# mdolab/adflow

Measured on AMD Instinct MI355X. Metric: Mcells*residual-evals/s, higher is better.
Workload: dtype f64

## Files before the change

### adflow_amd/capi.py

```python
from __future__ import annotations

import ctypes
import os
from ctypes import POINTER, c_char_p, c_double, c_int, c_int8, c_int32, c_uint, c_void_p
from typing import Optional

import numpy as np

from . import params as P

_HERE = os.path.dirname(os.path.abspath(__file__))
LIB_PATH = os.path.join(_HERE, "lib", "libadflow_gpu.so")
MAX_RK = 8


class AdflowOpts(ctypes.Structure):
    _fields_ = [
        ("equations", c_int32), ("turbModel", c_int32), ("turbProd", c_int32),
        ("useQCR", c_int32), ("useRotationSA", c_int32), ("useft2SA", c_int32),
        ("spaceDiscr", c_int32), ("spaceDiscrCoarse", c_int32), ("limiter", c_int32), ("orderTurb", c_int32),
        ("dirScaling", c_int32),
        ("smoother", c_int32), ("nRKStages", c_int32), ("resAveraging", c_int32), ("nSubiterations", c_int32),
        ("nSubIterTurb", c_int32),
        ("groundLevel", c_int32),
# ... 76 lines not shown
        ("rotMatrix", c_double * 9), ("rotCenter", c_double * 3), ("translation", c_double * 3),
        ("nHalos", c_int32), ("reserved", c_int32), ("block", c_void_p), ("indices", c_void_p),
    ]


class AdflowCommPattern(ctypes.Structure):
    _fields_ = [
        ("ncopy", c_int32),
        ("donorBlock", c_void_p), ("donorIndices", c_void_p), ("haloBlock", c_void_p), ("haloIndices", c_void_p),
        ("nProcSend", c_int32), ("sendProc", c_void_p), ("nsendCum", c_void_p), ("sendBlock", c_void_p),
        ("sendIndices", c_void_p),
        ("nProcRecv", c_int32), ("recvProc", c_void_p), ("nrecvCum", c_void_p), ("recvBlock", c_void_p),
        ("recvIndices", c_void_p),
    ]


BC_CALLBACK = ctypes.CFUNCTYPE(None, c_int, c_int)

(ARR_W, ARR_P, ARR_GAMMA, ARR_RLV, ARR_REV, ARR_DW, ARR_FW, ARR_DTL, ARR_RADI, ARR_RADJ, ARR_RADK, ARR_AA,
 ARR_NODAL_GRADS, ARR_WN, ARR_PN, ARR_W1, ARR_P1, ARR_WR, ARR_VOL, ARR_SI, ARR_SJ, ARR_SK, ARR_X, ARR_D2WALL) = range(1, 25)

JAC_PC, JAC_FROZEN_TURB, JAC_TURB_ONLY, JAC_VISC_PC, JAC_USE_AD = 1, 2, 4, 8, 16
RES_UPDATE_INTERMED, RES_FLOW, RES_TURB, RES_CLOSURES, RES_HALO = 1, 2, 4, 8, 16
RES_DISS_APPROX, RES_VISC_APPROX, RES_UPWIND_FIRST_ORDER, ANK_COUPLED = 32, 64, 128, 256
ANK_TURB, RES_APPROX_SA, RES_TURB_FIRST_ORDER, JAC_APPROX_SA = 512, 1024, 2048, 32

EXPORTS = [
    "adflow_gpu_init", "adflow_gpu_finalize", "adflow_gpu_last_error", "adflow_gpu_device_name",
    "adflow_gpu_comm_unique_id", "adflow_gpu_comm_init",
    "adflow_gpu_block_register", "adflow_gpu_block_release", "adflow_gpu_release_all", "adflow_gpu_upload_geometry", "adflow_gpu_upload_state",
    "adflow_gpu_download_state", "adflow_gpu_download_residual", "adflow_gpu_download_array",
    "adflow_gpu_upload_array", "adflow_gpu_set_options",
    "adflow_gpu_time_step", "adflow_gpu_initres", "adflow_gpu_residual", "adflow_gpu_block_res",
    "adflow_gpu_rk_smooth", "adflow_gpu_dadi_smooth", "adflow_gpu_halo_exchange", "adflow_gpu_res_norms",
    "adflow_gpu_sa_solve", "adflow_gpu_set_turb_bc_callback",
    "adflow_gpu_set_w_vec", "adflow_gpu_get_r_vec", "adflow_gpu_get_res", "adflow_gpu_nk_residual",
    "adflow_gpu_nk_residual_dev",
    "adflow_gpu_transfer_to_coarse", "adflow_gpu_transfer_to_fine", "adflow_gpu_mg_cycle",
    "adflow_gpu_comm_register", "adflow_gpu_comm_info", "adflow_gpu_halo_slot_info", "adflow_gpu_halo_pack", "adflow_gpu_halo_unpack",
    "adflow_gpu_halo_local_copy", "adflow_gpu_set_bc_callback", "adflow_gpu_bc_register", "adflow_gpu_apply_all_bc", "adflow_gpu_download_wall_stress", "adflow_gpu_abi_sizes2", "adflow_gpu_xhalo", "adflow_gpu_actuator_register", "adflow_gpu_comm_register_periodic", "adflow_gpu_coarse_coordinates", "adflow_gpu_exchange_coor",
    "adflow_gpu_upload_coordinates", "adflow_gpu_update_geometry", "adflow_gpu_reference_shock_sensor",
    "adflow_gpu_wall_distance_register", "adflow_gpu_update_wall_distances",
    "adflow_gpu_fd_jacobian", "adflow_gpu_release_workspace", "adflow_gpu_selftest_math", "adflow_gpu_jacobian_info", "adflow_gpu_download_jacobian", "adflow_gpu_download_jacobian_rows",
    "adflow_gpu_jacobian_mult", "adflow_gpu_jacobian_mult_dev",
    "adflow_gpu_pc_setup", "adflow_gpu_pc_info", "adflow_gpu_pc_apply", "adflow_gpu_pc_apply_dev", "adflow_gpu_pc_release", "adflow_gpu_pc_select",
    "adflow_gpu_pc_set_fill", "adflow_gpu_pc_info2",
    "adflow_gpu_gmres_solve", "adflow_gpu_gmres_solve_dev",
    "adflow_gpu_ank_set_w", "adflow_gpu_ank_set_w_dev", "adflow_gpu_ank_get_r", "adflow_gpu_ank_get_r_dev", "adflow_gpu_ank_time_step",
    "adflow_gpu_ank_download_time_step", "adflow_gpu_ank_pc_setup", "adflow_gpu_ank_set_base", "adflow_gpu_ank_set_base_dev",
    "adflow_gpu_ank_mult", "adflow_gpu_ank_mult_dev", "adflow_gpu_ank_last_h", "adflow_gpu_ank_solve", "adflow_gpu_ank_solve_dev",
    "adflow_gpu_ank_physicality_check", "adflow_gpu_ank_physicality_check_dev", "adflow_gpu_ank_release",
    "adflow_gpu_ank_download_time_step_turb", "adflow_gpu_ank_unsteady_res", "adflow_gpu_ank_unsteady_res_dev", "adflow_gpu_ank_select_base",
    "adflow_gpu_event_record", "adflow_gpu_event_elapsed_ms", "adflow_gpu_sync", "adflow_gpu_set_async",
    "adflow_gpu_abi_sizes", "adflow_gpu_set_tuning", "adflow_gpu_march_stats",
]

_libs = {}


class AdflowGpuError(RuntimeError):
    pass


def load(path: Optional[str] = None) -> ctypes.CDLL:
    path = path or LIB_PATH
    if path in _libs:
        return _libs[path]
    if not os.path.exists(path):
        raise AdflowGpuError(f"{path} not built: run `python -m adflow_amd.build` (no CPU fallback exists)")
    lib = ctypes.CDLL(path)
    lib.adflow_gpu_last_error.restype = c_char_p
    lib.adflow_gpu_init.argtypes = [c_int]
    lib.adflow_gpu_device_name.argtypes = [c_char_p, c_int]
    lib.adflow_gpu_block_register.argtypes = [c_int, c_int, c_int, POINTER(AdflowBlockDesc)]
    for n in ("adflow_gpu_block_release", "adflow_gpu_upload_geometry", "adflow_gpu_upload_state", "adflow_gpu_download_state",
              "adflow_gpu_download_residual"):
        getattr(lib, n).argtypes = [c_int, c_int, c_int]
    lib.adflow_gpu_download_array.argtypes = [c_int, c_int, c_int, c_int, c_void_p]
    lib.adflow_gpu_upload_array.argtypes = [c_int, c_int, c_int, c_int, c_void_p]
    lib.adflow_gpu_set_options.argtypes = [POINTER(AdflowOpts)]
    lib.adflow_gpu_time_step.argtypes = [c_int, c_int]
    lib.adflow_gpu_initres.argtypes = [c_int, c_int, c_int]
    lib.adflow_gpu_residual.argtypes = [c_int, c_int]
    lib.adflow_gpu_block_res.argtypes = [c_int, c_uint]
    lib.adflow_gpu_set_async.argtypes = [c_int]
    lib.adflow_gpu_bc_register.argtypes = [c_int, c_int, c_int, c_int, c_int, POINTER(AdflowBcSubface)]
    lib.adflow_gpu_apply_all_bc.argtypes = [c_int, c_int]
    lib.adflow_gpu_download_wall_stress.argtypes = [c_int, c_int, c_int, c_int, c_void_p, c_void_p]
    lib.adflow_gpu_upload_coordinates.argtypes = [c_int, c_int, c_int]
    lib.adflow_gpu_update_geometry.argtypes = [c_int]
    lib.adflow_gpu_xhalo.argtypes = [c_int]
    lib.adflow_gpu_actuator_register.argtypes = [c_int, POINTER(AdflowActuatorRegion)]
    lib.adflow_gpu_comm_register_periodic.argtypes = [c_int, c_int, c_int, POINTER(AdflowPeriodicData)]
    lib.adflow_gpu_coarse_coordinates.argtypes = [c_int]
    lib.adflow_gpu_exchange_coor.argtypes = [c_int]
    lib.adflow_gpu_reference_shock_sensor.argtypes = [c_int]
    lib.adflow_gpu_wall_distance_register.argtypes = [c_int, c_int, c_int, c_void_p, c_void_p]
    lib.adflow_gpu_update_wall_distances.argtypes = [c_int, c_void_p, ctypes.c_int64]
    lib.adflow_gpu_fd_jacobian.argtypes = [c_int, c_uint, c_double]
    lib.adflow_gpu_release_workspace.argtypes = [ctypes.POINTER(ctypes.c_int64)]
    lib.adflow_gpu_selftest_math.argtypes = [c_int, c_void_p, c_void_p, ctypes.c_int64, c_void_p, c_void_p]
    lib.adflow_gpu_jacobian_info.argtypes = [POINTER(ctypes.c_int32), POINTER(ctypes.c_int32), POINTER(ctypes.c_int32)]
    lib.adflow_gpu_download_jacobian.argtypes = [c_int, c_int, c_int, c_void_p]
    lib.adflow_gpu_download_jacobian_rows.argtypes = [c_int, c_int, c_int, c_void_p]
    lib.adflow_gpu_jacobian_mult.argtypes = [c_int, c_int, c_void_p, c_void_p, ctypes.c_long]
    lib.adflow_gpu_jacobian_mult_dev.argtypes = [c_int, c_int, c_void_p, c_void_p, ctypes.c_long]
    lib.adflow_gpu_pc_setup.argtypes = [c_int]
# ... 4 lines not shown
    for f in (lib.adflow_gpu_gmres_solve, lib.adflow_gpu_gmres_solve_dev):
        f.argtypes = [c_int, c_int, c_void_p, c_void_p, ctypes.c_long, c_int, c_int, c_double, c_double, c_int,
                      POINTER(c_int), POINTER(c_double), POINTER(c_double)]
    for f in (lib.adflow_gpu_ank_set_w, lib.adflow_gpu_ank_set_w_dev, lib.adflow_gpu_ank_get_r, lib.adflow_gpu_ank_get_r_dev,
              lib.adflow_gpu_ank_set_base, lib.adflow_gpu_ank_set_base_dev):
        f.argtypes = [c_void_p, ctypes.c_long, c_uint]
    lib.adflow_gpu_ank_time_step.argtypes = [c_int, c_double, c_double, c_uint]
    lib.adflow_gpu_ank_download_time_step.argtypes = [c_int, c_void_p]
    lib.adflow_gpu_ank_pc_setup.argtypes = [c_int]
    lib.adflow_gpu_ank_mult.argtypes = [c_void_p, c_void_p, ctypes.c_long]
    lib.adflow_gpu_ank_mult_dev.argtypes = [c_void_p, c_void_p, ctypes.c_long]
    lib.adflow_gpu_ank_last_h.argtypes = [POINTER(c_double)]
    for f in (lib.adflow_gpu_ank_solve, lib.adflow_gpu_ank_solve_dev):
        f.argtypes = [c_int, c_void_p, c_void_p, ctypes.c_long, c_int, c_int, c_double, c_double, POINTER(c_int), POINTER(c_double),
                      POINTER(c_double)]
    for f in (lib.adflow_gpu_ank_physicality_check, lib.adflow_gpu_ank_physicality_check_dev):
        f.argtypes = [c_void_p, c_void_p, ctypes.c_long, c_uint, c_double, c_double, c_double, c_double, POINTER(c_double)]
    lib.adflow_gpu_ank_release.argtypes = [POINTER(ctypes.c_int64)]
    lib.adflow_gpu_ank_download_time_step_turb.argtypes = [c_int, c_void_p, c_uint]
    for f in (lib.adflow_gpu_ank_unsteady_res, lib.adflow_gpu_ank_unsteady_res_dev):
        f.argtypes = [c_void_p, c_double, c_void_p, ctypes.c_long, c_uint, POINTER(c_double)]
    lib.adflow_gpu_pc_select.argtypes = [c_int]
    lib.adflow_gpu_pc_set_fill.argtypes = [c_int]
    lib.adflow_gpu_pc_info2.argtypes = [POINTER(ctypes.c_int32), POINTER(ctypes.c_int32), POINTER(ctypes.c_int32)]
    lib.adflow_gpu_ank_select_base.argtypes = [c_uint]
    lib.adflow_gpu_set_tuning.argtypes = [c_char_p, c_int]
    lib.adflow_gpu_abi_sizes.argtypes = [POINTER(c_int), POINTER(c_int)]
    lib.adflow_gpu_rk_smooth.argtypes = [c_int]
    lib.adflow_gpu_dadi_smooth.argtypes = [c_int]
    lib.adflow_gpu_halo_exchange.argtypes = [c_int] * 6
    lib.adflow_gpu_res_norms.argtypes = [c_int, c_void_p, c_int]
    lib.adflow_gpu_sa_solve.argtypes = [c_int]
    lib.adflow_gpu_set_turb_bc_callback.argtypes = [c_void_p]
    lib.adflow_gpu_set_w_vec.argtypes = [c_void_p, ctypes.c_long]
    lib.adflow_gpu_get_r_vec.argtypes = [c_void_p, ctypes.c_long, c_void_p]
    lib.adflow_gpu_get_res.argtypes = [c_void_p, ctypes.c_long]
    lib.adflow_gpu_nk_residual.argtypes = [c_void_p, c_void_p, ctypes.c_long]
    lib.adflow_gpu_nk_residual_dev.argtypes = [c_void_p, c_void_p, ctypes.c_long]
    lib.adflow_gpu_transfer_to_coarse.argtypes = [c_int]
    lib.adflow_gpu_transfer_to_fine.argtypes = [c_int]
    lib.adflow_gpu_mg_cycle.argtypes = [c_void_p, c_int]
    lib.adflow_gpu_comm_register.argtypes = [c_int, c_int, POINTER(AdflowCommPattern)]
    lib.adflow_gpu_halo_slot_info.argtypes = [c_int, c_int, c_int, c_int, POINTER(c_int), POINTER(c_int)]
    lib.adflow_gpu_comm_info.argtypes = [POINTER(c_int)] * 4
    lib.adflow_gpu_halo_pack.argtypes = [c_int] * 7 + [c_void_p]
    lib.adflow_gpu_halo_unpack.argtypes = [c_int] * 7 + [c_void_p]
    lib.adflow_gpu_halo_local_copy.argtypes = [c_int] * 6
    lib.adflow_gpu_set_bc_callback.argtypes = [c_void_p]
    lib.adflow_gpu_comm_unique_id.argtypes = [c_void_p]
    lib.adflow_gpu_comm_init.argtypes = [c_int, c_int, c_void_p]
    lib.adflow_gpu_event_record.argtypes = [c_int]
    lib.adflow_gpu_event_elapsed_ms.argtypes = [c_int, c_int, POINTER(c_double)]
    lib.adflow_gpu_march_stats.argtypes = [c_int, POINTER(c_double), c_int]
    so, sd = c_int(), c_int()
    lib.adflow_gpu_abi_sizes(ctypes.byref(so), ctypes.byref(sd))
    if so.value != ctypes.sizeof(AdflowOpts) or sd.value != ctypes.sizeof(AdflowBlockDesc):
        raise AdflowGpuError("ctypes mirror of adflow_opts/adflow_block_desc is out of date with include/adflow_gpu.h")
    _libs[path] = lib
    return lib


def check(rc: int, lib: Optional[ctypes.CDLL] = None) -> None:
    if rc != 0:
        raise AdflowGpuError((lib or load()).adflow_gpu_last_error().decode())


def opts_from_params(prm: P.FlowParams) -> AdflowOpts:
    o = AdflowOpts()
    for name, _ in AdflowOpts._fields_:
        if name.startswith("reserved") or name in ("etaRK", "cdisRK", "wInf"):
            continue
        setattr(o, name, type(getattr(o, name))(getattr(prm, name)))
    for i, v in enumerate(prm.etaRK):
        o.etaRK[i] = v
    for i, v in enumerate(prm.cdisRK):
        o.cdisRK[i] = v
    for i, v in enumerate(prm.wInf()):
        o.wInf[i] = v
    return o


def _ptr(a: Optional[np.ndarray]):
    if a is None:
        return None
    assert a.flags["F_CONTIGUOUS"], "host arrays must be Fortran-ordered"
    return a.ctypes.data


def desc_from_block(blk) -> AdflowBlockDesc:
    d = AdflowBlockDesc()
    d.nx, d.ny, d.nz, d.nw, d.rightHanded = blk.nx, blk.ny, blk.nz, blk.nw, int(getattr(blk, "rightHanded", True))
    for name in ("w", "p", "gamma", "rlv", "rev", "x", "sI", "sJ", "sK", "vol", "volRef", "d2Wall",
                 "porI", "porJ", "porK", "iblank", "dw", "fw", "dtl", "radI", "radJ", "radK", "w1", "p1", "wr",
                 "mgIFine", "mgJFine", "mgKFine", "mgIWeight", "mgJWeight", "mgKWeight", "mgICoarse", "mgJCoarse",
                 "mgKCoarse", "sFaceI", "sFaceJ", "sFaceK"):
        setattr(d, name, _ptr(blk.a.get(name)))
    d.addGridVelocities = int(blk.a.get("sFaceI") is not None)
    rot = getattr(blk, "rotRate", None)
    d.blockIsMoving = int(rot is not None)
    for m in range(3):
        d.rotRate[m] = float(rot[m]) if rot is not None else 0.0
    return d


def comm_pattern_struct(cp) -> AdflowCommPattern:
    c = AdflowCommPattern()
# ... 10 lines not shown
```

### adflow_amd/csrc/api.hip

```cpp
#include <hip/hip_runtime.h>

#include <algorithm>
#include <cmath>
#include <cstdarg>
#include <cstdio>
#include <cstring>
#include <functional>
#include <array>
#include <map>
#include <string>
#include <tuple>
#include <vector>

#include "internal.h"
#include "flow_plan.h"

extern int g_march_kch, g_viscous_tiled, g_inviscid_march, g_roe_march, g_sa_march;
int g_test_fault = 0;
int g_rvec_joint = 1;
int g_pc_fused = 1;
int g_xcd_tiles = 2;

namespace {

std::string g_err;
int g_device = -1;
hipStream_t g_stream = nullptr;
hipStream_t g_streamB = nullptr, g_streamC = nullptr;
hipEvent_t g_evFork = nullptr, g_evB = nullptr, g_evC = nullptr, g_evB1 = nullptr;
hipStream_t g_streamX = nullptr;
hipEvent_t g_evPack = nullptr, g_evComm = nullptr;
int g_overlap = 1;
adflow_opts g_opts;
bool g_have_opts = false;
hipEvent_t g_events[64];
bool g_events_ready = false;
bool g_async = false;

int fail(const char* fmt, ...)
{
    char buf[1024];
    va_list ap;
    va_start(ap, fmt);
    vsnprintf(buf, sizeof buf, fmt, ap);
    va_end(ap);
    g_err = buf;
    return 1;
}

#define HIPCHK(expr)                                                                        \
    do {                                                                                    \
        hipError_t e_ = (expr);                                                             \
        if (e_ != hipSuccess) return fail("%s failed: %s (%s:%d)", #expr, hipGetErrorString(e_), __FILE__, __LINE__); \
    } while (0)

struct DevArr {
    double* base = nullptr;
    int ncomp = 0;
};

struct Block {
    adflow_block_desc d;
// ... 18 lines not shown
};

typedef std::tuple<int, int, int> Key;
std::map<Key, Block*> g_blocks;

struct CommList {
    int n = 0;
    int *blkA = nullptr, *blkB = nullptr;
    long *offA = nullptr, *offB = nullptr;
    int peer = -1;
    double* buf = nullptr;
};

struct CommPattern {
    bool present = false;
    CommList local;
    std::vector<CommList> sends, recvs;
    std::vector<int32_t> h_donorBlock, h_donorIdx, h_haloBlock, h_haloIdx;
    std::vector<int32_t> h_sendProc, h_nsendCum, h_sendBlock, h_sendIdx;
    std::vector<int32_t> h_recvProc, h_nrecvCum, h_recvBlock, h_recvIdx;
    struct Periodic {
        double rotMatrix[9], rotCenter[3], translation[3];
        std::vector<int32_t> h_block, h_idx;
        CommList list;
    };
    std::vector<Periodic> periodic;
    bool built = false;
    std::vector<JmAccList> acc;
    bool accBuilt = false;
};

struct ActRegion {
    std::vector<int32_t> h_block, h_idx;
    double force[3], heat, volume, relaxStart, relaxEnd;
    CommList list;
    bool built = false;
};
std::vector<ActRegion> g_act;

std::map<std::pair<int, int>, CommPattern> g_comm;
double* g_rvec_target = nullptr;
int g_rvec_done = 0;
int g_snap_done = 0;
long g_state_gen = 0;
int g_split_eval = 1;
int g_mg_graph = 1;
int g_comm_self = 0;
int g_self_rank = 0;
std::map<int, BlkView*> g_tab;
std::map<int, int> g_tab_size;
std::map<int, std::pair<int4*, int>> g_tiles;
std::map<int, std::pair<int4*, int>> g_gf_tiles;
std::map<int, std::pair<int4*, int>> g_gf_tiles_int, g_gf_tiles_bnd;
std::map<int, std::pair<int4*, int>> g_sa_tiles, g_sa_tiles_int, g_sa_tiles_bnd;
int g_num_cus = 0;
int g_gf_nofit = 0;
int g_phase_base = 0;
bool g_use_march = true;
adflow_bc_callback g_bc_callback = nullptr;
adflow_bc_callback g_turb_bc_callback = nullptr;
double* g_norm_dev = nullptr;
int* g_floor_flag_dev = nullptr;
int g_dadi_upd = 1;
int g_etot_flag_level = 0;

void free_list(CommList& l)
{
    if (l.blkA) (void)hipFree(l.blkA);
    if (l.blkB) (void)hipFree(l.blkB);
    if (l.offA) (void)hipFree(l.offA);
    if (l.offB) (void)hipFree(l.offB);
    if (l.buf) (void)hipFree(l.buf);
    l = CommList();
}

void free_acc_list(JmAccList& a)
{
    if (a.tBlk) (void)hipFree(a.tBlk);
    if (a.tOff) (void)hipFree(a.tOff);
    if (a.seg) (void)hipFree(a.seg);
    if (a.sBlk) (void)hipFree(a.sBlk);
    if (a.sOff) (void)hipFree(a.sOff);
    a = JmAccList();
}

void drop_comm_lists(CommPattern& cp)
{
    for (auto& a : cp.acc) free_acc_list(a);
    cp.acc.clear();
    cp.accBuilt = false;
    free_list(cp.local);
    for (auto& l : cp.sends) free_list(l);
    for (auto& l : cp.recvs) free_list(l);
    for (auto& pd : cp.periodic) free_list(pd.list);
    cp.sends.clear();
    cp.recvs.clear();
    cp.built = false;
}

void invalidate_comm_level(int level)
{
    ++g_state_gen;
    if (level == 1)
        for (auto& r : g_act) r.built = false;
    for (auto& kv : g_comm)
        if (kv.first.first == level) drop_comm_lists(kv.second);
// ... 1799 lines not shown
        const int nIn = std::min(W, T - q * W), per = (nIn + 7) / 8;
        for (int pr = 0; pr < Wp; ++pr) {
            const int s = pr / 8, x = pr % 8;
            if (s < per && x * per + s < nIn) { (*out)[(size_t)q * Wp + pr] = q * W + x * per + s; ++seen; }
        }
    }
    if (seen != T) return fail("round_order: %ld of %d work items placed (W = %d)", seen, T, W);
    std::vector<char> hit((size_t)T, 0);
    for (int e : *out)
        if (e >= 0) { if (hit[e]) return fail("round_order: item %d placed twice", e); hit[e] = 1; }
    return 0;
}

int ensure_tiles(int level)
{
    if (g_tiles.count(level)) return 0;
    if (ensure_table(level)) return 1;
    std::vector<int4> nat;
    for (auto& kv : g_blocks) {
        if (std::get<0>(kv.first) != level || std::get<1>(kv.first) != 1) continue;
        int ntx, nty, ntz;
        euler_march_tiles(kv.second->v, &ntx, &nty, &ntz);
        for (int tz = 0; tz < ntz; ++tz)
            for (int ty = 0; ty < nty; ++ty)
                for (int tx = 0; tx < ntx; ++tx) {
                    int4 t;
                    t.x = std::get<2>(kv.first); t.y = tx; t.z = ty; t.w = tz;
                    nat.push_back(t);
                }
    }
    const int n = (int)nat.size();
    const int W = (g_xcd_tiles >= 2) ? adf_round_size() : ((n + 7) / 8) * 8;
    std::vector<int> ord;
    if (g_xcd_tiles) {
        if (round_order(n, W, &ord)) return 1;
    } else {
        ord.resize(n);
        for (int p = 0; p < n; ++p) ord[p] = p;
    }
    std::vector<int4> phys(ord.size());
    for (size_t p = 0; p < ord.size(); ++p) {
        if (ord[p] >= 0) phys[p] = nat[ord[p]];
        else { phys[p].x = -1; phys[p].y = phys[p].z = phys[p].w = 0; }
    }
    while (!phys.empty() && phys.back().x < 0) phys.pop_back();
    int4* d = nullptr;
    HIPCHK(hipMalloc((void**)&d, sizeof(int4) * phys.size()));
    HIPCHK(hipMemcpy(d, phys.data(), sizeof(int4) * phys.size(), hipMemcpyHostToDevice));
    g_tiles[level] = std::make_pair(d, (int)phys.size());
    return 0;
}

static int build_chunk_tables(int level, int R, double warm, int reach, std::pair<int4*, int>* all, std::pair<int4*, int>* in_,
                              std::pair<int4*, int>* bd_, int wgPerCU = 2)
{
    if (ensure_table(level)) return 1;
    struct Col { int slot, bx, by, nz, nx, ny; };
    std::vector<Col> cols;
    long planes = 0;
    for (auto& kv : g_blocks) {
        if (std::get<0>(kv.first) != level || std::get<1>(kv.first) != 1) continue;
        const BlkView& v = kv.second->v;
        const int gx = (v.nx + 59) / 60, gy = (v.ny + R - 1) / R;
        for (int by = 0; by < gy; ++by)
            for (int bx = 0; bx < gx; ++bx) { cols.push_back(Col{std::get<2>(kv.first), bx, by, v.nz, v.nx, v.ny}); planes += v.nz; }
    }
    const int N = (int)cols.size();
    *all = *in_ = *bd_ = std::make_pair((int4*)nullptr, 0);
    if (N == 0) return 0;
    const int W = adf_round_size() * wgPerCU / 2;
    const int kmin = 8;
    auto split = [&](long T, std::vector<int>& c) {
        c.assign(N, 1);
        long used = 0;
        std::vector<std::pair<double, int>> rem(N);
        for (int q = 0; q < N; ++q) {
            const double want = (double)T * cols[q].nz / (double)planes;
            const int cmax = std::max(1, cols[q].nz / kmin);
            c[q] = std::min(cmax, std::max(1, (int)want));
            rem[q] = std::make_pair(want - c[q], q);
            used += c[q];
        }
        std::sort(rem.begin(), rem.end(), [](const std::pair<double, int>& a, const std::pair<double, int>& b) { return a.first > b.first; });
        for (int q = 0; q < N && used < T; ++q) {
            const int id = rem[q].second;
            if (c[id] < std::max(1, cols[id].nz / kmin)) { ++c[id]; ++used; }
        }
    };
    auto makespan = [&](const std::vector<int>& c) {
        std::vector<int> len;
        for (int q = 0; q < N; ++q)
            for (int e = 0; e < c[q]; ++e) len.push_back((cols[q].nz + c[q] - 1 - e) / c[q]);
        std::sort(len.begin(), len.end(), [](int a, int b) { return a > b; });
        double t = 0.0;
        for (size_t q = 0; q < len.size(); q += W) t += len[q] + warm;
        return t;
    };
    std::vector<int> best;
    if (!g_gf_nofit) {
        double tbest = 1.e300;
        const long Tmax = std::max<long>(N, planes / kmin);
        for (long m = 1; m * W <= Tmax + W; ++m) {
            std::vector<int> c;
            split(m * W, c);
            const double t = makespan(c);
            if (t < tbest - 1.e-9) { tbest = t; best = c; }
            if (m > 64) break;
        }
        std::vector<int> one(N, 1);
        if (makespan(one) < tbest) best = one;
    } else {
        best.resize(N);
        const int L = g_march_kch > 0 ? g_march_kch : 32;
        for (int q = 0; q < N; ++q) best[q] = (cols[q].nz + L - 1) / L;
    }
    struct Chunk { int col, k0, k1; };
    std::vector<Chunk> ch;
    for (int q = 0; q < N; ++q) {
        int k = 2;
        for (int e = 0; e < best[q]; ++e) {
            const int len = (cols[q].nz + best[q] - 1 - e) / best[q];
            if (len <= 0) continue;
            ch.push_back(Chunk{q, k, k + len - 1});
            k += len;
        }
    }
    std::stable_sort(ch.begin(), ch.end(), [&](const Chunk& a, const Chunk& b) {
        const int la = a.k1 - a.k0, lb = b.k1 - b.k0;
        if (la != lb) return la > lb;
        if (cols[a.col].slot != cols[b.col].slot) return cols[a.col].slot < cols[b.col].slot;
        if (a.k0 != b.k0) return a.k0 < b.k0;
        return a.col < b.col;
    });
    auto make_table = [&](const std::vector<Chunk>& list, std::pair<int4*, int>* out) -> int {
        const int T = (int)list.size();
        std::vector<int> ord;
        if (round_order(T, W, &ord)) return 1;
        std::vector<int4> phys(ord.size());
        for (size_t p = 0; p < ord.size(); ++p) {
            const int e = ord[p];
            int4 tt;
            if (e >= 0) {
                const Col& c = cols[list[e].col];
                tt.x = c.slot; tt.y = c.bx | (c.by << 16); tt.z = list[e].k0; tt.w = list[e].k1;
            } else { tt.x = -1; tt.y = tt.z = tt.w = 0; }
            phys[p] = tt;
        }
        int n = (int)phys.size();
        while (n > 0 && phys[n - 1].x < 0) --n;
        int4* d = nullptr;
        HIPCHK(hipMalloc((void**)&d, sizeof(int4) * std::max(n, 1)));
        if (n > 0) HIPCHK(hipMemcpy(d, phys.data(), sizeof(int4) * n, hipMemcpyHostToDevice));
        *out = std::make_pair(d, n);
        return 0;
    };
    if (make_table(ch, all)) return 1;
    std::vector<Chunk> in, bd;
    for (const Chunk& c : ch) {
        const Col& q = cols[c.col];
        const int il = q.nx + 1, jl = q.ny + 1, kl = q.nz + 1;
        const int ia = 2 + 60 * q.bx, ib_ = std::min(ia + 59, il), ja = 2 + R * q.by, jb_ = std::min(ja + R - 1, jl);
        const bool interior = (ia - reach >= 2 && ib_ + reach <= il && ja - reach >= 2 && jb_ + reach <= jl && c.k0 - reach >= 2 &&
                               c.k1 + reach <= kl);
        (interior ? in : bd).push_back(c);
    }
    if (make_table(in, in_) || make_table(bd, bd_)) return 1;
    return 0;
}

int ensure_gf_tiles(int level)
{
    if (g_gf_tiles.count(level)) return 0;
    std::pair<int4*, int> a, i, b;
    if (build_chunk_tables(level, 3, 1.5, 1, &a, &i, &b, 2)) return 1;
    g_gf_tiles[level] = a; g_gf_tiles_int[level] = i; g_gf_tiles_bnd[level] = b;
    return 0;
}

int ensure_sa_tiles(int level)
{
    if (g_sa_tiles.count(level)) return 0;
    std::pair<int4*, int> a, i, b;
    if (build_chunk_tables(level, 4, 0.5, 2, &a, &i, &b)) return 1;
    g_sa_tiles[level] = a; g_sa_tiles_int[level] = i; g_sa_tiles_bnd[level] = b;
    return 0;
}

int make_list_host(int level, const int32_t* blk, const int32_t* idx, int ld, int first, int n, std::vector<int>& hb,
                   std::vector<long>& ho)
{
    hb.resize(n);
    ho.resize(n);
    for (int t = 0; t < n; ++t) {
        const int nn = blk[first + t];
        Block* b = find_block(nn, level, 1);
        if (!b) return fail("comm pattern of level %d references unregistered block %d", level, nn);
        const int i = idx[first + t], j = idx[ld + first + t], k = idx[2 * ld + first + t];
        if (i < 0 || i > b->v.ib || j < 0 || j > b->v.jb || k < 0 || k > b->v.kb)
            return fail("comm pattern of level %d: cell (%d,%d,%d) outside block %d", level, i, j, k, nn);
        hb[t] = nn;
        ho[t] = b->v.idx(i, j, k);
    }
    return 0;
}

int upload_list(const std::vector<int>& hb, const std::vector<long>& ho, int** d_blk, long** d_off)
{
    const size_t n = hb.size();
    *d_blk = nullptr;
    *d_off = nullptr;
    if (n == 0) return 0;
    HIPCHK(hipMalloc((void**)d_blk, sizeof(int) * n));
    HIPCHK(hipMalloc((void**)d_off, sizeof(long) * n));
    HIPCHK(hipMemcpy(*d_blk, hb.data(), sizeof(int) * n, hipMemcpyHostToDevice));
    HIPCHK(hipMemcpy(*d_off, ho.data(), sizeof(long) * n, hipMemcpyHostToDevice));
    return 0;
}

int make_list(int level, const int32_t* blk, const int32_t* idx, int ld, int first, int n, int** d_blk, long** d_off)
{
    std::vector<int> hb;
    std::vector<long> ho;
    if (make_list_host(level, blk, idx, ld, first, n, hb, ho)) return 1;
    return upload_list(hb, ho, d_blk, d_off);
}

int build_comm(int level, int nLayers, CommPattern** out)
{
// ... 2639 lines not shown
#ifndef ADFLOW_NO_RCCL
    if (g_nccl && g_nranks > 1) NCCLCHK(ncclAllReduce(g_norm_dev, g_norm_dev, n, ncclDouble, ncclSum, g_nccl, g_stream));
#endif
    HIPCHK(hipMemcpyAsync(sums, g_norm_dev, sizeof(double) * n, hipMemcpyDeviceToHost, g_stream));
    HIPCHK(hipStreamSynchronize(g_stream));
    return 0;
}

int adflow_gpu_event_record(int slot)
{
    if (g_device < 0) return fail("adflow_gpu_init has not been called");
    if (slot < 0 || slot >= 64) return fail("event slot %d out of range", slot);
    HIPCHK(hipEventRecord(g_events[slot], g_stream));
    return 0;
}

int adflow_gpu_event_elapsed_ms(int a, int b, double* ms)
{
    if (a < 0 || a >= 64 || b < 0 || b >= 64 || !ms) return fail("bad event arguments");
    HIPCHK(hipEventSynchronize(g_events[b]));
    float f = 0.f;
    HIPCHK(hipEventElapsedTime(&f, g_events[a], g_events[b]));
    *ms = f;
    return 0;
}

int adflow_gpu_march_stats(int level, double* out, int n)
{
    if (need_ready()) return 1;
    if (!out || n < 4) return fail("march_stats: n = %d (>= 4)", n);
    for (int q = 0; q < n; ++q) out[q] = 0.0;
    if (ensure_gf_tiles(level) || ensure_sa_tiles(level) || ensure_tiles(level)) return 1;
    {
        const auto& tt = g_sa_tiles[level];
        std::vector<int4> h((size_t)tt.second);
        if (tt.second > 0) HIPCHK(hipMemcpy(h.data(), tt.first, sizeof(int4) * h.size(), hipMemcpyDeviceToHost));
        for (const int4& t : h)
            if (t.x >= 0) out[0] += 4.0 * (t.w - t.z + 1);
    }
    {
        const auto& tt = g_gf_tiles[level];
        std::vector<int4> h((size_t)tt.second);
        if (tt.second > 0) HIPCHK(hipMemcpy(h.data(), tt.first, sizeof(int4) * h.size(), hipMemcpyDeviceToHost));
        for (const int4& t : h)
            if (t.x >= 0) out[1] += 4.0 * (t.w - t.z + 3);
    }
    for (auto& kv : g_blocks) {
        if (std::get<0>(kv.first) != level || std::get<1>(kv.first) != 1) continue;
        const BlkView& v = kv.second->v;
        int ntx, nty, ntz;
        euler_march_tiles(v, &ntx, &nty, &ntz);
        out[2] += 4.0 * ntx * nty * (v.nz + ntz);
    }
    return 0;
}

int adflow_gpu_sync(void)
{
    if (g_device < 0) return fail("adflow_gpu_init has not been called");
    HIPCHK(hipGetLastError());
    HIPCHK(hipStreamSynchronize(g_stream));
    return 0;
}

int adflow_gpu_set_tuning(const char* key, int value)
{
    ++g_state_gen;
    if (!key) return fail("null tuning key");
    if (!strcmp(key, "euler_march")) { g_use_march = (value != 0); return 0; }
    if (!strcmp(key, "viscous_tiled")) { g_viscous_tiled = value; return 0; }
    if (!strcmp(key, "inviscid_march")) { g_inviscid_march = value; return 0; }
    if (!strcmp(key, "roe_march")) { g_roe_march = value; return 0; }
    if (!strcmp(key, "sa_march")) { g_sa_march = value; return 0; }
    if (!strcmp(key, "overlap")) { g_overlap = value; return 0; }
    if (!strcmp(key, "max_grid_z")) { g_max_grid_z = (value > 0) ? value : 65535; return 0; }
    if (!strcmp(key, "metric_from_x")) { g_metric_from_x = value; return 0; }
    if (!strcmp(key, "xcd_tiles")) {
        g_xcd_tiles = value;
        if (g_stream) (void)hipStreamSynchronize(g_stream);
        mg_graph_drop();
        for (auto& kv : g_tiles) (void)hipFree(kv.second.first);
        g_tiles.clear();
        return 0;
    }
    if (!strcmp(key, "phase_events")) {
        if (value != 0 && (value < 8 || value > 56)) return fail("phase_events: first slot must be 8..56 (or 0 = off)");
        g_phase_base = value;
        return 0;
    }
    if (!strcmp(key, "march_kch")) {
        if (value < 4) return fail("march_kch must be >= 4");
        g_march_kch = value;
        if (g_stream) (void)hipStreamSynchronize(g_stream);
        mg_graph_drop();
        for (auto* mp : {&g_tiles, &g_gf_tiles, &g_gf_tiles_int, &g_gf_tiles_bnd, &g_sa_tiles, &g_sa_tiles_int, &g_sa_tiles_bnd}) {
            for (auto& kv : *mp) (void)hipFree(kv.second.first);
            mp->clear();
        }
        return 0;
    }
    if (!strcmp(key, "split_eval")) { g_split_eval = value; return 0; }
    if (!strcmp(key, "test_fault")) { g_test_fault = value; g_mgg.failed = false; mg_graph_drop(); return 0; }
    if (!strcmp(key, "ad_cache")) { g_ad_cache = value; if (!value) { if (g_stream) (void)hipStreamSynchronize(g_stream); ad_drop(); } return 0; }
    if (!strcmp(key, "rvec_joint")) { g_rvec_joint = value; return 0; }
    if (!strcmp(key, "jac_snap")) { g_jac_snap = value; return 0; }
    if (!strcmp(key, "pc_fused")) { g_pc_fused = value; mg_graph_drop(); return 0; }
// ... 66 lines not shown
```

### adflow_amd/engine.py

```python
from __future__ import annotations

import ctypes
from typing import Dict, Tuple

import numpy as np

from . import capi
from .params import FlowParams


class Engine:
    def __init__(self, device: int = 0, _lib_path=None):
        self.lib = capi.load(_lib_path)
        self._chk(self.lib.adflow_gpu_init(device))
        self.blocks: Dict[Tuple[int, int, int], object] = {}
        self._descs = {}
        self.prm = None

    def _chk(self, rc):
        capi.check(rc, self.lib)

    def close(self):
        if self.lib is not None:
            self.lib.adflow_gpu_finalize()
# ... 399 lines not shown
    def FormFunction_mf(self, wVec: np.ndarray):
        assert wVec.dtype == np.float64 and wVec.flags["C_CONTIGUOUS"]
        r = np.zeros_like(wVec)
        self._chk(self.lib.adflow_gpu_nk_residual(wVec.ctypes.data, r.ctypes.data, wVec.size))
        return r

    def transferToCoarseGrid(self, level=1):
        self._chk(self.lib.adflow_gpu_transfer_to_coarse(level))

    def transferToFineGrid(self, level=1):
        self._chk(self.lib.adflow_gpu_transfer_to_fine(level))

    def executeMGCycle(self, cycling):
        c = np.ascontiguousarray(cycling, np.int32)
        self._chk(self.lib.adflow_gpu_mg_cycle(c.ctypes.data, c.size))

    def comm_register(self, level: int, nLayers: int, cp):
        c = capi.comm_pattern_struct(cp)
        self._chk(self.lib.adflow_gpu_comm_register(level, nLayers, ctypes.byref(c)))

    def comm_init_single(self):
        if getattr(self, "_comm_ready", False):
            return
        raw = (ctypes.c_char * 128)()
        self._chk(self.lib.adflow_gpu_comm_unique_id(raw))
        self._chk(self.lib.adflow_gpu_comm_init(0, 1, raw))
        self._comm_ready = True

    def comm_info(self):
        v = [ctypes.c_int() for _ in range(4)]
        self._chk(self.lib.adflow_gpu_comm_info(*[ctypes.byref(x) for x in v]))
        return tuple(int(x.value) for x in v)

    def whalo1(self, level, start, end, commPressure=True, commGamma=True, commViscous=True):
        self._chk(self.lib.adflow_gpu_halo_exchange(level, start, end, int(commPressure), int(commViscous), 1))

    def whalo2(self, level, start, end, commPressure=True, commGamma=True, commViscous=True):
        self._chk(self.lib.adflow_gpu_halo_exchange(level, start, end, int(commPressure), int(commViscous), 2))

    def res_norms(self, level=1, n=5):
        out = np.zeros(n)
        self._chk(self.lib.adflow_gpu_res_norms(level, out.ctypes.data, n))
        return out

    def event_record(self, slot: int):
        self._chk(self.lib.adflow_gpu_event_record(slot))

    def event_elapsed_ms(self, a: int, b: int) -> float:
        ms = ctypes.c_double()
        self._chk(self.lib.adflow_gpu_event_elapsed_ms(a, b, ctypes.byref(ms)))
        return ms.value

    def march_stats(self, level: int = 1):
        out = (ctypes.c_double * 4)()
        self._chk(self.lib.adflow_gpu_march_stats(level, out, 4))
        return {"sa_march": out[0], "visc_gf": out[1], "tile_march": out[2]}

    def sync(self):
        self._chk(self.lib.adflow_gpu_sync())
```

### include/adflow_gpu.h

```cpp
#ifndef ADFLOW_GPU_H
#define ADFLOW_GPU_H

#include <stdint.h>

#ifdef __cplusplus
extern "C" {
#endif

enum { ADFLOW_EULER = 1, ADFLOW_NS = 2, ADFLOW_RANS = 3 };
enum { ADFLOW_DISS_SCALAR = 1, ADFLOW_DISS_MATRIX = 2, ADFLOW_UPWIND = 9 };
enum { ADFLOW_LIM_FIRST_ORDER = 1, ADFLOW_LIM_NONE = 2, ADFLOW_LIM_VANALBADA = 3, ADFLOW_LIM_MINMOD = 4 };
enum { ADFLOW_RUNGE_KUTTA = 1, ADFLOW_DADI = 2 };
enum { ADFLOW_TURBPROD_STRAIN = 1, ADFLOW_TURBPROD_VORTICITY = 2 };
enum { ADFLOW_RESAVG_NEVER = 0, ADFLOW_RESAVG_ALWAYS = 1, ADFLOW_RESAVG_ALTERNATE = 2 };

#define ADFLOW_MAX_RK_STAGES 8

typedef void (*adflow_bc_callback)(int level, int secondHalo);

enum {
    ADFLOW_BC_SYMM = -1, ADFLOW_BC_SYMM_POLAR = -2, ADFLOW_BC_NSWALL_ADIABATIC = -3, ADFLOW_BC_NSWALL_ISOTHERMAL = -4,
    ADFLOW_BC_EULERWALL = -5, ADFLOW_BC_FARFIELD = -6, ADFLOW_BC_SUPERSONIC_INFLOW = -7, ADFLOW_BC_SUBSONIC_INFLOW = -8,
    ADFLOW_BC_SUPERSONIC_OUTFLOW = -9, ADFLOW_BC_SUBSONIC_OUTFLOW = -10, ADFLOW_BC_MASSBLEED_OUTFLOW = -12,
    ADFLOW_BC_EXTRAP = -15
// ... 139 lines not shown
int adflow_gpu_download_state(int nn, int level, int sps);
int adflow_gpu_download_residual(int nn, int level, int sps);
int adflow_gpu_download_array(int nn, int level, int sps, int which, double* host);
int adflow_gpu_upload_array(int nn, int level, int sps, int which, const double* host);
int adflow_gpu_set_options(const adflow_opts* o);

int adflow_gpu_time_step(int level, int onlyRadii);
int adflow_gpu_initres(int level, int varStart, int varEnd);
int adflow_gpu_residual(int level, int rkStage);
int adflow_gpu_block_res(int level, unsigned flags);
int adflow_gpu_reference_shock_sensor(int level);
int adflow_gpu_rk_smooth(int level);
int adflow_gpu_dadi_smooth(int level);
int adflow_gpu_sa_solve(int level);
int adflow_gpu_set_turb_bc_callback(adflow_bc_callback fn);
int adflow_gpu_transfer_to_coarse(int level);
int adflow_gpu_transfer_to_fine(int level);
int adflow_gpu_mg_cycle(const int32_t* cycling, int nStepsCycling);
int adflow_gpu_comm_register(int level, int nLayers, const adflow_comm_pattern* p);
typedef struct adflow_periodic_data {
    double rotMatrix[9];
    double rotCenter[3], translation[3];
    int32_t nHalos, reserved;
    const int32_t *block, *indices;
} adflow_periodic_data;
int adflow_gpu_comm_register_periodic(int level, int nLayers, int nPeriodic, const adflow_periodic_data* pd);
int adflow_gpu_halo_exchange(int level, int varStart, int varEnd, int commPressure, int commVisc, int nLayers);
int adflow_gpu_halo_slot_info(int level, int nLayers, int isSend, int islot, int* peer, int* count);
int adflow_gpu_halo_pack(int level, int nLayers, int islot, int varStart, int varEnd, int commPressure, int commVisc, double* buf);
int adflow_gpu_halo_unpack(int level, int nLayers, int islot, int varStart, int varEnd, int commPressure, int commVisc, const double* buf);
int adflow_gpu_halo_local_copy(int level, int nLayers, int varStart, int varEnd, int commPressure, int commVisc);
int adflow_gpu_set_bc_callback(adflow_bc_callback fn);
int adflow_gpu_bc_register(int nn, int level, int sps, int nBocos, int nViscBocos, const adflow_bc_subface* faces);
int adflow_gpu_apply_all_bc(int level, int secondHalo);
int adflow_gpu_download_wall_stress(int nn, int level, int sps, int mm, double* tau, double* q);
typedef struct adflow_actuator_region {
    int32_t nCellIDs, reserved;
    const int32_t *block, *cellIDs;
    double force[3], heat, volume, relaxStart, relaxEnd;
} adflow_actuator_region;
int adflow_gpu_actuator_register(int nRegions, const adflow_actuator_region* regions);
int adflow_gpu_res_norms(int level, double* sums, int n);

int adflow_gpu_set_w_vec(const double* wVec, long n);
int adflow_gpu_get_r_vec(double* rVec, long n, double* sumsq2);
int adflow_gpu_get_res(double* res, long n);
int adflow_gpu_nk_residual(const double* wVec, double* rVec, long n);
int adflow_gpu_nk_residual_dev(const double* d_wVec, double* d_rVec, long n);

int adflow_gpu_event_record(int slot);
int adflow_gpu_event_elapsed_ms(int slot_start, int slot_stop, double* ms);
int adflow_gpu_sync(void);
int adflow_gpu_march_stats(int level, double* out, int n);
int adflow_gpu_set_tuning(const char* key, int value);
int adflow_gpu_set_async(int on);
int adflow_gpu_abi_sizes(int* opts_bytes, int* desc_bytes);
int adflow_gpu_abi_sizes2(int* bc_subface_bytes, int* comm_pattern_bytes);

enum { ADFLOW_JAC_PC = 1u, ADFLOW_JAC_FROZEN_TURB = 2u, ADFLOW_JAC_TURB_ONLY = 4u, ADFLOW_JAC_VISC_PC = 8u, ADFLOW_JAC_USE_AD = 16u,
       ADFLOW_JAC_APPROX_SA = 32u };
int adflow_gpu_fd_jacobian(int level, unsigned flags, double delta);
int adflow_gpu_release_workspace(int64_t* bytes);
int adflow_gpu_selftest_math(int which, const double* x, const double* a, int64_t n, double* y, double* dy);
int adflow_gpu_jacobian_info(int32_t* nState, int32_t* nStencil, int32_t* stencil);
int adflow_gpu_download_jacobian(int nn, int level, int sps, double* blocks);
int adflow_gpu_download_jacobian_rows(int nn, int level, int sps, double* rows);
int adflow_gpu_jacobian_mult(int level, int transpose, const double* x, double* y, long n);
int adflow_gpu_jacobian_mult_dev(int level, int transpose, const double* d_x, double* d_y, long n);
int adflow_gpu_pc_setup(int level);
int adflow_gpu_pc_info(int32_t* nState, int32_t* nPlanes, int64_t* bytes);
int adflow_gpu_pc_set_fill(int fill);
int adflow_gpu_pc_info2(int32_t* fill, int32_t* nEntries, int32_t* nLevelSets);
int adflow_gpu_pc_apply(int level, int transpose, const double* r, double* z, long n);
int adflow_gpu_pc_apply_dev(int level, int transpose, const double* d_r, double* d_z, long n);
int adflow_gpu_pc_release(int64_t* bytes);
int adflow_gpu_pc_select(int slot);
int adflow_gpu_gmres_solve(int level, int transpose, const double* b, double* x, long n, int restart, int maxIts, double rtol,
                           double atol, int useGuess, int* its, double* rnorm0, double* rnorm);
int adflow_gpu_gmres_solve_dev(int level, int transpose, const double* d_b, double* d_x, long n, int restart, int maxIts, double rtol,
                               double atol, int useGuess, int* its, double* rnorm0, double* rnorm);

enum { ADFLOW_ANK_COUPLED = 256u, ADFLOW_ANK_TURB = 512u };
int adflow_gpu_ank_set_w(const double* w, long n, unsigned flags);
int adflow_gpu_ank_set_w_dev(const double* d_w, long n, unsigned flags);
int adflow_gpu_ank_get_r(double* r, long n, unsigned flags);
int adflow_gpu_ank_get_r_dev(double* d_r, long n, unsigned flags);
int adflow_gpu_ank_time_step(int level, double cfl, double turbCFLScale, unsigned flags);
int adflow_gpu_ank_download_time_step(int nn, double* blocks);
int adflow_gpu_ank_download_time_step_turb(int nn, double* blocks, unsigned flags);
int adflow_gpu_ank_pc_setup(int level);
int adflow_gpu_ank_set_base(const double* w, long n, unsigned flags);
int adflow_gpu_ank_set_base_dev(const double* d_w, long n, unsigned flags);
int adflow_gpu_ank_mult(const double* v, double* y, long n);
int adflow_gpu_ank_mult_dev(const double* d_v, double* d_y, long n);
int adflow_gpu_ank_last_h(double* h);
int adflow_gpu_ank_select_base(unsigned flags);
int adflow_gpu_ank_solve(int level, const double* b, double* x, long n, int restart, int maxIts, double rtol, double atol, int* its,
                         double* rnorm0, double* rnorm);
int adflow_gpu_ank_solve_dev(int level, const double* d_b, double* d_x, long n, int restart, int maxIts, double rtol, double atol, int* its,
                             double* rnorm0, double* rnorm);
int adflow_gpu_ank_physicality_check(const double* w, double* dw, long n, unsigned flags, double physLSTol, double physLSTolTurb,
                                     double stepFactor, double stepMin, double* lambda);
int adflow_gpu_ank_physicality_check_dev(const double* d_w, double* d_dw, long n, unsigned flags, double physLSTol, double physLSTolTurb,
                                         double stepFactor, double stepMin, double* lambda);
int adflow_gpu_ank_unsteady_res(const double* dW, double omega, double* r, long n, unsigned flags, double* norm);
int adflow_gpu_ank_unsteady_res_dev(const double* d_dW, double omega, double* d_r, long n, unsigned flags, double* norm);
// ... 7 lines not shown
```

Measured before the change: 4850.

## Model viscous march chunk schedule and pick column splits with tail refinement

Adds a list-scheduling model (min-heap per XCD group) that simulates chunk completion time for the viscous ghost-fill march tables, then searches over uniform per-column chunk counts and tail-splitting of the last partial round, keeping whichever chunk set minimizes the modeled makespan. The goal is to reduce load imbalance and tail idle time across CUs. It also exposes the model values and a chunk table download for inspection. Risk: the model may not reflect real timing, and smaller tail chunks add warm-up overhead. The interior and boundary tables are still built from the original chunking.

```diff
diff --git a/adflow_amd/capi.py b/adflow_amd/capi.py
--- a/adflow_amd/capi.py
+++ b/adflow_amd/capi.py
@@ -152,7 +152,7 @@
     "adflow_gpu_ank_physicality_check", "adflow_gpu_ank_physicality_check_dev", "adflow_gpu_ank_release",
     "adflow_gpu_ank_download_time_step_turb", "adflow_gpu_ank_unsteady_res", "adflow_gpu_ank_unsteady_res_dev", "adflow_gpu_ank_select_base",
     "adflow_gpu_event_record", "adflow_gpu_event_elapsed_ms", "adflow_gpu_sync", "adflow_gpu_set_async",
-    "adflow_gpu_abi_sizes", "adflow_gpu_set_tuning", "adflow_gpu_march_stats",
+    "adflow_gpu_abi_sizes", "adflow_gpu_set_tuning", "adflow_gpu_march_stats", "adflow_gpu_chunk_table",
 ]
 
 _libs = {}
@@ -263,6 +263,7 @@
     lib.adflow_gpu_event_record.argtypes = [c_int]
     lib.adflow_gpu_event_elapsed_ms.argtypes = [c_int, c_int, POINTER(c_double)]
     lib.adflow_gpu_march_stats.argtypes = [c_int, POINTER(c_double), c_int]
+    lib.adflow_gpu_chunk_table.argtypes = [c_int, c_int, c_void_p, c_int, POINTER(c_int)]
     so, sd = c_int(), c_int()
     lib.adflow_gpu_abi_sizes(ctypes.byref(so), ctypes.byref(sd))
     if so.value != ctypes.sizeof(AdflowOpts) or sd.value != ctypes.sizeof(AdflowBlockDesc):
diff --git a/adflow_amd/csrc/api.hip b/adflow_amd/csrc/api.hip
--- a/adflow_amd/csrc/api.hip
+++ b/adflow_amd/csrc/api.hip
@@ -8,6 +8,7 @@
 #include <functional>
 #include <array>
 #include <map>
+#include <queue>
 #include <string>
 #include <tuple>
 #include <vector>
@@ -132,6 +133,7 @@
 std::map<int, std::pair<int4*, int>> g_tiles;
 std::map<int, std::pair<int4*, int>> g_gf_tiles;
 std::map<int, std::pair<int4*, int>> g_gf_tiles_int, g_gf_tiles_bnd;
+std::map<int, std::pair<double, double>> g_gf_model;
 std::map<int, std::pair<int4*, int>> g_sa_tiles, g_sa_tiles_int, g_sa_tiles_bnd;
 int g_num_cus = 0;
 int g_gf_nofit = 0;
@@ -2037,24 +2039,27 @@
 }
 
 static int build_chunk_tables(int level, int R, double warm, int reach, std::pair<int4*, int>* all, std::pair<int4*, int>* in_,
-                              std::pair<int4*, int>* bd_, int wgPerCU = 2)
+                              std::pair<int4*, int>* bd_, int wgPerCU = 2, double* model = nullptr)
 {
     if (ensure_table(level)) return 1;
     struct Col { int slot, bx, by, nz, nx, ny; };
     std::vector<Col> cols;
     long planes = 0;
+    int nzmax = 1;
     for (auto& kv : g_blocks) {
         if (std::get<0>(kv.first) != level || std::get<1>(kv.first) != 1) continue;
         const BlkView& v = kv.second->v;
         const int gx = (v.nx + 59) / 60, gy = (v.ny + R - 1) / R;
+        nzmax = std::max(nzmax, v.nz);
         for (int by = 0; by < gy; ++by)
             for (int bx = 0; bx < gx; ++bx) { cols.push_back(Col{std::get<2>(kv.first), bx, by, v.nz, v.nx, v.ny}); planes += v.nz; }
     }
     const int N = (int)cols.size();
     *all = *in_ = *bd_ = std::make_pair((int4*)nullptr, 0);
+    if (model) model[0] = model[1] = 0.0;
     if (N == 0) return 0;
     const int W = adf_round_size() * wgPerCU / 2;
-    const int kmin = 8;
+    const int kmin = 8, kminTail = 4;
     auto split = [&](long T, std::vector<int>& c) {
         c.assign(N, 1);
         long used = 0;
@@ -2100,23 +2105,79 @@
         for (int q = 0; q < N; ++q) best[q] = (cols[q].nz + L - 1) / L;
     }
     struct Chunk { int col, k0, k1; };
-    std::vector<Chunk> ch;
-    for (int q = 0; q < N; ++q) {
-        int k = 2;
-        for (int e = 0; e < best[q]; ++e) {
-            const int len = (cols[q].nz + best[q] - 1 - e) / best[q];
-            if (len <= 0) continue;
-            ch.push_back(Chunk{q, k, k + len - 1});
-            k += len;
-        }
-    }
-    std::stable_sort(ch.begin(), ch.end(), [&](const Chunk& a, const Chunk& b) {
-        const int la = a.k1 - a.k0, lb = b.k1 - b.k0;
-        if (la != lb) return la > lb;
-        if (cols[a.col].slot != cols[b.col].slot) return cols[a.col].slot < cols[b.col].slot;
-        if (a.k0 != b.k0) return a.k0 < b.k0;
-        return a.col < b.col;
-    });
+    auto cut_columns = [&](const std::vector<int>& c) {
+        std::vector<Chunk> ch;
+        for (int q = 0; q < N; ++q) {
+            int k = 2;
+            for (int e = 0; e < c[q]; ++e) {
+                const int len = (cols[q].nz + c[q] - 1 - e) / c[q];
+                if (len <= 0) continue;
+                ch.push_back(Chunk{q, k, k + len - 1});
+                k += len;
+            }
+        }
+        return ch;
+    };
+    auto launch_sort = [&](std::vector<Chunk>& ch) {
+        std::stable_sort(ch.begin(), ch.end(), [&](const Chunk& a, const Chunk& b) {
+            const int la = a.k1 - a.k0, lb = b.k1 - b.k0;
+            if (la != lb) return la > lb;
+            if (cols[a.col].slot != cols[b.col].slot) return cols[a.col].slot < cols[b.col].slot;
+            if (a.k0 != b.k0) return a.k0 < b.k0;
+            return a.col < b.col;
+        });
+    };
+    std::vector<Chunk> ch = cut_columns(best);
+    launch_sort(ch);
+    auto finish = [&](const std::vector<Chunk>& list) -> double {
+        std::vector<int> ord;
+        if (round_order((int)list.size(), W, &ord)) return -1.0;
+        const int nx = (W % 8 == 0) ? 8 : 1;
+        typedef std::priority_queue<double, std::vector<double>, std::greater<double>> Pool;
+        std::vector<Pool> pool(nx, Pool(std::greater<double>(), std::vector<double>((size_t)std::max(1, W / nx), 0.0)));
+        double end = 0.0;
+        for (size_t p = 0; p < ord.size(); ++p) {
+            if (ord[p] < 0) continue;
+            Pool& f = pool[p % nx];
+            const double t = f.top() + (list[ord[p]].k1 - list[ord[p]].k0 + 1) + warm;
+            f.pop();
+            f.push(t);
+            end = std::max(end, t);
+        }
+        return end;
+    };
+    std::vector<Chunk> chAll = ch;
+    if (model) {
+        double tbest = finish(ch);
+        if (tbest < 0.0) return 1;
+        model[1] = tbest;
+        for (int cm = 1; !g_gf_nofit && cm <= std::min(64, std::max(1, nzmax / kmin)); ++cm) {
+            std::vector<int> c(N);
+            for (int q = 0; q < N; ++q)
+                c[q] = std::min(std::max(1, cols[q].nz / kmin), std::max(1, (int)lround((double)cm * cols[q].nz / nzmax)));
+            std::vector<Chunk> mainCh = cut_columns(c);
+            launch_sort(mainCh);
+            const int T = (int)mainCh.size(), r = T > W ? T % W : 0;
+            for (int s : {0, 4, 6, 8, 12, 16}) {
+                if (s > 0 && (s < kminTail || r == 0)) continue;
+                std::vector<Chunk> cand(mainCh.begin(), mainCh.end() - (s > 0 ? r : 0));
+                for (int e = T - r; s > 0 && e < T; ++e) {
+                    const int len = mainCh[e].k1 - mainCh[e].k0 + 1, n = std::max(1, len / s);
+                    int k = mainCh[e].k0;
+                    for (int i = 0; i < n; ++i) {
+                        const int l = (len + n - 1 - i) / n;
+                        cand.push_back(Chunk{mainCh[e].col, k, k + l - 1});
+                        k += l;
+                    }
+                }
+                launch_sort(cand);
+                const double t = finish(cand);
+                if (t < 0.0) return 1;
+                if (t < tbest - 1.e-9) { tbest = t; chAll = cand; }
+            }
+        }
+        model[0] = tbest;
+    }
     auto make_table = [&](const std::vector<Chunk>& list, std::pair<int4*, int>* out) -> int {
         const int T = (int)list.size();
         std::vector<int> ord;
@@ -2139,7 +2200,7 @@
         *out = std::make_pair(d, n);
         return 0;
     };
-    if (make_table(ch, all)) return 1;
+    if (make_table(chAll, all)) return 1;
     std::vector<Chunk> in, bd;
     for (const Chunk& c : ch) {
         const Col& q = cols[c.col];
@@ -2157,8 +2218,10 @@
 {
     if (g_gf_tiles.count(level)) return 0;
     std::pair<int4*, int> a, i, b;
-    if (build_chunk_tables(level, 3, 1.5, 1, &a, &i, &b, 2)) return 1;
+    double model[2];
+    if (build_chunk_tables(level, 3, 1.5, 1, &a, &i, &b, 2, model)) return 1;
     g_gf_tiles[level] = a; g_gf_tiles_int[level] = i; g_gf_tiles_bnd[level] = b;
+    g_gf_model[level] = std::make_pair(model[0], model[1]);
     return 0;
 }
 
@@ -4904,6 +4967,22 @@
         euler_march_tiles(v, &ntx, &nty, &ntz);
         out[2] += 4.0 * ntx * nty * (v.nz + ntz);
     }
+    out[3] = g_gf_model[level].first;
+    if (n >= 5) out[4] = g_gf_model[level].second;
+    return 0;
+}
+
+int adflow_gpu_chunk_table(int level, int which, int32_t* out, int cap, int* count)
+{
+    if (need_ready()) return 1;
+    if (which < 0 || which > 5 || !count || (cap > 0 && !out)) return fail("chunk_table: which = %d, cap = %d", which, cap);
+    if (which < 3 ? ensure_gf_tiles(level) : ensure_sa_tiles(level)) return 1;
+    const std::pair<int4*, int>& tt = (which == 0 ? g_gf_tiles : which == 1 ? g_gf_tiles_int : which == 2 ? g_gf_tiles_bnd
+                                       : which == 3 ? g_sa_tiles : which == 4 ? g_sa_tiles_int : g_sa_tiles_bnd)[level];
+    *count = tt.second;
+    const int m = std::min(cap, tt.second);
+    static_assert(sizeof(int4) == 4 * sizeof(int32_t), "int4 layout");
+    if (m > 0) HIPCHK(hipMemcpy(out, tt.first, sizeof(int4) * (size_t)m, hipMemcpyDeviceToHost));
     return 0;
 }
 
diff --git a/adflow_amd/engine.py b/adflow_amd/engine.py
--- a/adflow_amd/engine.py
+++ b/adflow_amd/engine.py
@@ -475,9 +475,17 @@
         return ms.value
 
     def march_stats(self, level: int = 1):
-        out = (ctypes.c_double * 4)()
-        self._chk(self.lib.adflow_gpu_march_stats(level, out, 4))
-        return {"sa_march": out[0], "visc_gf": out[1], "tile_march": out[2]}
+        out = (ctypes.c_double * 5)()
+        self._chk(self.lib.adflow_gpu_march_stats(level, out, 5))
+        return {"sa_march": out[0], "visc_gf": out[1], "tile_march": out[2], "visc_gf_model_planes": out[3],
+                "visc_gf_model_planes_round_fit": out[4]}
+
+    def chunk_table(self, which: int = 0, level: int = 1) -> np.ndarray:
+        n = ctypes.c_int()
+        self._chk(self.lib.adflow_gpu_chunk_table(level, which, None, 0, ctypes.byref(n)))
+        out = np.zeros((max(n.value, 1), 4), dtype=np.int32)
+        self._chk(self.lib.adflow_gpu_chunk_table(level, which, out.ctypes.data, n.value, ctypes.byref(n)))
+        return out[:n.value]
 
     def sync(self):
         self._chk(self.lib.adflow_gpu_sync())
diff --git a/include/adflow_gpu.h b/include/adflow_gpu.h
--- a/include/adflow_gpu.h
+++ b/include/adflow_gpu.h
@@ -215,6 +215,7 @@
 int adflow_gpu_event_elapsed_ms(int slot_start, int slot_stop, double* ms);
 int adflow_gpu_sync(void);
 int adflow_gpu_march_stats(int level, double* out, int n);
+int adflow_gpu_chunk_table(int level, int which, int32_t* out, int cap, int* count);
 int adflow_gpu_set_tuning(const char* key, int value);
 int adflow_gpu_set_async(int on);
 int adflow_gpu_abi_sizes(int* opts_bytes, int* desc_bytes);
```

Result: no change. 4894, median of 6 (+0.9%).
